# Image-Processing-Systems-Laboratory/DeepInPainting

Measured on AMD Instinct MI355X. Metric: train images/sec at 256x256, batch 8/GPU, 1/2/4/8 MI355X; IPSR layer ms, higher is better.
Workload: dtype f32; 1 GPU; BASELINE config 2: 256x256 synthetic images, 128x128 centre mask (M=256 of N=1024 feature positions), batch 8/GPU, fp32, full IPSR training step; global_batch=8, parallelism=dp1, dropout=True, conv_math=fp32, vgg16=seeded random init (no pretrained weights offline)

## Files before the change

### deepinpainting_amd/csrc/ipsr_common.h

```cpp
#pragma once
#include <hip/hip_runtime.h>
#include <stddef.h>
#include <stdint.h>

#include "../../include/ipsr_hip.h"

namespace ipsr {

void set_error(const char* fmt, ...);
int fail(int code, const char* fmt, ...);
int check_launch(const char* what);

void profile_mark_start(hipStream_t st, int region = 0);
void profile_mark_stop(hipStream_t st, int region = 0, double work = 0.0, double work2 = 0.0);

int debug_option(int key);

static inline size_t align_up(size_t v, size_t a) { return (v + a - 1) / a * a; }
static inline int cdiv(int a, int b) { return (a + b - 1) / b; }

struct Carver {
    char* base;
    size_t off;
    size_t cap;
    explicit Carver(void* p, size_t bytes) : base(static_cast<char*>(p)), off(0), cap(bytes) {}
    template <typename T>
    T* take(size_t count) {
        size_t start = align_up(off, 256);
        off = start + count * sizeof(T);
        return reinterpret_cast<T*>(base + start);
    }
    bool ok() const { return off <= cap; }
};

__device__ __forceinline__ unsigned xcd_remap(unsigned wg, unsigned nwg)
{
    const unsigned q = nwg >> 3, r = nwg & 7u;
    const unsigned xcd = wg & 7u, slot = wg >> 3;
    const unsigned start = xcd < r ? xcd * (q + 1u) : r * (q + 1u) + (xcd - r) * q;
    return start + slot;
}

__device__ __forceinline__ void remap2d(bool on, unsigned& bx, unsigned& by)
{
    bx = blockIdx.x; by = blockIdx.y;
    if (on) {
        const unsigned L = xcd_remap(blockIdx.x + gridDim.x * blockIdx.y, gridDim.x * gridDim.y);
        by = L / gridDim.x; bx = L - by * gridDim.x;
    }
}

struct CorrPartials {
    const float* pval;
    const int32_t* pidx;
    int ksplit;
};

__device__ __forceinline__ bool better(float v1, int i1, float v0, int i0)
{
    const bool n1 = v1 != v1, n0 = v0 != v0;
    return (v1 > v0) || (n1 && !n0) || ((v1 == v0 || (n1 && n0)) && i1 < i0);
}
__device__ __forceinline__ bool takes_over(float v, float best) { return (v > best) || (v != v && best == best); }

__device__ __forceinline__ void merged_argmax(const CorrPartials& cp, int b, int N, int q, float& v, int& i)
{
    const size_t base = (size_t)b * cp.ksplit * N + q;
    v = cp.pval[base];
    i = cp.pidx[base];
    for (int s = 1; s < cp.ksplit; ++s) {
        const float vs = cp.pval[base + (size_t)s * N];
        const int is = cp.pidx[base + (size_t)s * N];
        if (better(vs, is, v, i)) { v = vs; i = is; }
    }
    i = min(max(i, 0), N - 1);
}

typedef unsigned short bf16_t;
__device__ __forceinline__ float bf2f(bf16_t h) { return __uint_as_float((unsigned)h << 16); }
__device__ __forceinline__ bf16_t f2bf(float f)
{
    unsigned u = __float_as_uint(f);
    u += 0x7fffu + ((u >> 16) & 1u);
    return (bf16_t)(u >> 16);
}
__device__ __forceinline__ unsigned f2bf2(float lo, float hi) { return (unsigned)f2bf(lo) | ((unsigned)f2bf(hi) << 16); }
__device__ __forceinline__ float ld1(const float* p, size_t i) { return p[i]; }
__device__ __forceinline__ float ld1(const bf16_t* p, size_t i) { return bf2f(p[i]); }
__device__ __forceinline__ void st1(float* p, size_t i, float v) { p[i] = v; }
__device__ __forceinline__ void st1(bf16_t* p, size_t i, float v) { p[i] = f2bf(v); }
__device__ __forceinline__ float4 ld4(const float* p, size_t i4) { return reinterpret_cast<const float4*>(p)[i4]; }
__device__ __forceinline__ float4 ld4(const bf16_t* p, size_t i4)
{
    const uint2 r = reinterpret_cast<const uint2*>(p)[i4];
    return make_float4(__uint_as_float(r.x << 16), __uint_as_float(r.x & 0xffff0000u), __uint_as_float(r.y << 16),
                       __uint_as_float(r.y & 0xffff0000u));
}
__device__ __forceinline__ void st4(float* p, size_t i4, float4 v) { reinterpret_cast<float4*>(p)[i4] = v; }
__device__ __forceinline__ void st4(bf16_t* p, size_t i4, float4 v)
{
    uint2 r;
    r.x = (unsigned)f2bf(v.x) | ((unsigned)f2bf(v.y) << 16);
    r.y = (unsigned)f2bf(v.z) | ((unsigned)f2bf(v.w) << 16);
    reinterpret_cast<uint2*>(p)[i4] = r;
}

__device__ __forceinline__ int mpi_at(const int32_t* __restrict__ mpi, int l, int N)
{
    const int q = mpi[l];
    return q < 0 ? 0 : (q >= N ? N - 1 : q);
}

int launch_feat_mask(const uint8_t* mask, int H, int W, int layers, float threshold, uint8_t* feat,
                     void* ws, size_t ws_bytes, hipStream_t st);
int launch_index_prep(const uint8_t* feat, int h, int w, int patch, int stride, int mask_thred,
                      int32_t* flag, int32_t* mask_point_idx, int32_t* count, hipStream_t st);
int launch_patch_normalize(const float* x, int B, int C, int N, float* xn, float* xT, int Cp, float* inv,
                           hipStream_t st, int ldx = 0, int ldn = 0);
int launch_unfold(const float* x, int B, int C, int h, int w, int patch, int ld, float* xu, hipStream_t st);
int launch_fold(const float* yu, int B, int C, int h, int w, int patch, float* out, hipStream_t st, const float* addend = nullptr);
int launch_window_prepare(const float* x, int B, int C, int h, int w, int patch, float* n1, float* inv, float* xT, int Cp, hipStream_t st);
size_t window_corr_ws_bytes(int B, int Np);
int launch_window_corr_argmax(const float* R, const float* inv, int B, int h, int w, int patch, void* ws, size_t ws_bytes, hipStream_t st,
                              CorrPartials* partials);
size_t corr_argmax_ws_bytes(int B, int C, int N);
int launch_corr_argmax(const float* xn, const float* ref, int B, int C, int N, int32_t* ind, float* vmax,
                       float* S_out, void* ws, size_t ws_bytes, hipStream_t st, CorrPartials* partials = nullptr);

bool corr_bf16_supported(int C, int N);
size_t corr_argmax_bf16_ws_bytes(int B, int C, int N);
int launch_corr_argmax_bf16(const float* xn, const float* ref, int B, int C, int N, int32_t* ind, float* vmax,
                            void* ws, size_t ws_bytes, hipStream_t st, CorrPartials* partials = nullptr);
bool corr_R_bf16_supported(int C);
size_t corr_R_bf16_ws_bytes(int B, int C, int N);
int launch_corr_R_bf16(const float* x, const float* ref, int B, int C, int N, float* R, void* ws, size_t ws_bytes, hipStream_t st);

size_t conv_gemm_ws_bytes(int transposed, int B, int Cred, int M, int Hin, int Win, int Hout, int Wout, int k, int stride, int pad, int dil);
int launch_conv_gemm(bool transposed, bool w_cred_major, const float* x, const float* w, float* y, int B, int Cred, int M,
                     int Hin, int Win, int Hout, int Wout, int k, int stride, int pad, int dil, void* ws, size_t ws_bytes, hipStream_t st);

struct AttnArgs {
    const float* xT;
    const float* inv;
    int32_t* ind;
    float* vmax;
    CorrPartials part;
    const int32_t* mpi;
    int mpi_stride;
    const int32_t* mcount;
    int B, C, Cp, N, M, Mc;
    float* wn;
    float* wo;
    int32_t* kq;
    int32_t* jq;
    int32_t* dlist;
    int32_t* mprime;
    int32_t* rankflag;
    float* ac;
    float* attn;
    float* out;
    int32_t* bwd_index;
};
int launch_attention(const AttnArgs& a, hipStream_t st);
int attention_limits(int Cp, int N, int M, int Mc);

int launch_backward(const float* g, const int32_t* mpi, int M, const float* attn, const int32_t* bwd_index,
                    float triple_w, int B, int C, int N, float* gin, hipStream_t st, int identity = 1);

int launch_bias_act(void* x, const float* bias, int B, int C, int HW, int act, float slope, int io_bf16, void* y2, size_t y2_bstride,
                    unsigned* tickets, hipStream_t st);
int launch_bias_relu_pool2(const void* x, const float* bias, int B, int C, int H, int W, int io_bf16, void* y, hipStream_t st);
int launch_cat_relu_fwd(const void* y, const void* x, int B, int C1, int C2, int HW, int io_bf16, void* out, hipStream_t st);
int launch_cat_relu_bwd(const void* g, const void* out, int B, int C1, int C2, int HW, int io_bf16, void* dy, void* dx, hipStream_t st);

int launch_instnorm_act_fwd(const void* x, const float* bias, const float* gamma, const float* beta, float eps, int act, float slope,
                            int B, int C, int HW, int io_bf16, void* y, float* mean, float* rstd, size_t y_bstride, void* y2, size_t y2_bstride,
                            unsigned* tickets, hipStream_t st);
int launch_instnorm_act_bwd(const void* dy, const void* y, const void* x, const float* bias, const float* gamma, const float* mean,
                            const float* rstd, int act, float slope, int B, int C, int HW, int io_bf16, void* dx, float* dgamma_p,
                            float* dbeta_p, float* dbias_p, float* sums, unsigned* tickets, size_t dy_bstride, size_t y_bstride, const void* dy2,
                            size_t dy2_bstride, hipStream_t st);
int launch_bias_act_bwd(const void* dy, const void* y, int act, float slope, int B, int C, int HW, int io_bf16, void* dx, float* dbias_p,
                        float* sums, unsigned* tickets, const void* dy2, size_t dy2_bstride, hipStream_t st);

size_t innercos_ws_bytes(int B, int Cuse, int N);
int launch_innercos_loss(const float* x, int B, int Cx, int Cuse, int N, const float* mask, const float* target,
                         float strength, float* loss, void* ws, size_t ws_bytes, hipStream_t st);
int launch_innercos_loss_fused(const float* x, int B, int Cx, int Cuse, int N, const float* mask, const float* target, float strength, float* loss,
                               void* ws, size_t ws_bytes, unsigned* ticket, hipStream_t st);
int launch_innercos_backward(const float* x, int B, int Cx, int Cuse, int N, const float* mask,
                             const float* target, float strength, const float* grad_loss, float* grad_x,
                             hipStream_t st);

}
```

### deepinpainting_amd/csrc/winograd.hip

```cpp
#include <type_traits>

#include "ipsr_common.h"

namespace ipsr {

typedef float f32x16 __attribute__((ext_vector_type(16)));
typedef const __attribute__((address_space(1))) void* gptr_t;
typedef __attribute__((address_space(3))) void* lptr_t;

constexpr int WG_BM = 128, WG_BN = 128, WG_BK = 16, WG_NBUF = 4, WG_THREADS = 256;

struct WinoSplit {
    int nsplit, sps, xi_split, nsplit_t, sps_t;
    int nxi = 36;
    __host__ __device__ int slabs() const { return xi_split >= nxi ? nsplit : (xi_split <= 0 ? nsplit_t : (nsplit > nsplit_t ? nsplit : nsplit_t)); }
    __host__ __device__ int of(int xi) const { return xi < xi_split ? nsplit : nsplit_t; }
    __host__ __device__ int head_xi() const { return xi_split < nxi ? xi_split : nxi; }
    __host__ int workgroups(int tiles_per_xi) const { return tiles_per_xi * (head_xi() * nsplit + (nxi - head_xi()) * nsplit_t); }
};

__device__ __forceinline__ void wino_load_sum(const float* __restrict__ M, const WinoSplit sp, size_t plane, size_t off, float m[6][6])
{
#pragma unroll
    for (int i = 0; i < 6; ++i)
#pragma unroll
        for (int j = 0; j < 6; ++j) m[i][j] = M[(size_t)(i * 6 + j) * plane + off];
    const int nmin = sp.xi_split >= 36 ? sp.nsplit : (sp.nsplit < sp.nsplit_t ? sp.nsplit : sp.nsplit_t), nmax = sp.slabs();
    for (int s = 1; s < nmin; ++s) {
        const float* Ms = M + (size_t)s * 36 * plane;
#pragma unroll
        for (int i = 0; i < 6; ++i)
#pragma unroll
            for (int j = 0; j < 6; ++j) m[i][j] += Ms[(size_t)(i * 6 + j) * plane + off];
    }
    for (int s = nmin < 1 ? 1 : nmin; s < nmax; ++s) {
        const float* Ms = M + (size_t)s * 36 * plane;
#pragma unroll
        for (int i = 0; i < 6; ++i)
#pragma unroll
            for (int j = 0; j < 6; ++j)
                if (s < sp.of(i * 6 + j)) m[i][j] += Ms[(size_t)(i * 6 + j) * plane + off];
    }
}

__device__ __forceinline__ void wino_bt(const float d[6], float v[6])
{
    v[0] = 4.0f * d[0] - 5.0f * d[2] + d[4];
    v[1] = -4.0f * d[1] - 4.0f * d[2] + d[3] + d[4];
    v[2] = 4.0f * d[1] - 4.0f * d[2] - d[3] + d[4];
    v[3] = -2.0f * d[1] - d[2] + 2.0f * d[3] + d[4];
    v[4] = 2.0f * d[1] - d[2] - 2.0f * d[3] + d[4];
    v[5] = 4.0f * d[1] - 5.0f * d[3] + d[5];
}
__device__ __forceinline__ void wino_g(const float g[3], float u[6])
{
    u[0] = 0.25f * g[0];
    u[1] = (-1.0f / 6.0f) * (g[0] + g[1] + g[2]);
    u[2] = (-1.0f / 6.0f) * (g[0] - g[1] + g[2]);
    u[3] = (1.0f / 24.0f) * g[0] + (1.0f / 12.0f) * g[1] + (1.0f / 6.0f) * g[2];
    u[4] = (1.0f / 24.0f) * g[0] - (1.0f / 12.0f) * g[1] + (1.0f / 6.0f) * g[2];
    u[5] = g[2];
}
__device__ __forceinline__ void wino_at(const float m[6], float y[4])
{
    y[0] = m[0] + m[1] + m[2] + m[3] + m[4];
    y[1] = m[1] - m[2] + 2.0f * m[3] - 2.0f * m[4];
    y[2] = m[1] + m[2] + 4.0f * m[3] + 4.0f * m[4];
    y[3] = m[1] - m[2] + 8.0f * m[3] - 8.0f * m[4] + m[5];
}

__device__ __forceinline__ void wino_g4(const float e[4], float u[6])
{
    u[0] = 0.25f * e[0];
    u[1] = (-1.0f / 6.0f) * (e[0] + e[1] + e[2] + e[3]);
    u[2] = (-1.0f / 6.0f) * (e[0] - e[1] + e[2] - e[3]);
    u[3] = (1.0f / 24.0f) * e[0] + (1.0f / 12.0f) * e[1] + (1.0f / 6.0f) * e[2] + (1.0f / 3.0f) * e[3];
    u[4] = (1.0f / 24.0f) * e[0] - (1.0f / 12.0f) * e[1] + (1.0f / 6.0f) * e[2] - (1.0f / 3.0f) * e[3];
    u[5] = e[3];
}
__device__ __forceinline__ void wino_at3(const float m[6], float y[3])
{
    y[0] = m[0] + m[1] + m[2] + m[3] + m[4];
    y[1] = m[1] - m[2] + 2.0f * m[3] - 2.0f * m[4];
    y[2] = m[1] + m[2] + 4.0f * m[3] + 4.0f * m[4] + m[5];
}

typedef short bf16x8 __attribute__((ext_vector_type(8)));

constexpr int SPLIT_ROWS = 32;
constexpr int SPLIT_CHUNK = 12;
template <int NPL> constexpr int split_stage_elems() { return SPLIT_CHUNK * NPL * SPLIT_ROWS * 8; }

template <int NPL>
__device__ __forceinline__ void store_split(unsigned short* __restrict__ stage, const float (&v)[6][6], int pk, int rl,
                                            unsigned short* __restrict__ dst, size_t nblk, size_t rows, size_t blk, size_t row0)
{
    constexpr int NVEC = SPLIT_CHUNK * NPL * SPLIT_ROWS;
    const uint4* src = reinterpret_cast<const uint4*>(stage);
#pragma unroll
    for (int ch = 0; ch < 36 / SPLIT_CHUNK; ++ch) {
#pragma unroll
        for (int e = 0; e < SPLIT_CHUNK; ++e) {
            const int xi = ch * SPLIT_CHUNK + e;
            float r = v[xi / 6][xi % 6];
#pragma unroll
            for (int p = 0; p < NPL; ++p) {
                const unsigned short b = f2bf(r);
                stage[((e * NPL + p) * SPLIT_ROWS + rl) * 8 + pk] = b;
                r -= bf2f(b);
            }
        }
        __syncthreads();
#pragma unroll
        for (int it = 0; it < (NVEC + 255) / 256; ++it) {
            const int idx = threadIdx.x + it * 256;
            if (NVEC % 256 == 0 || idx < NVEC) {
                const int xp = idx / SPLIT_ROWS, r2 = idx - xp * SPLIT_ROWS;
                *reinterpret_cast<uint4*>(dst + (((size_t)(ch * SPLIT_CHUNK * NPL + xp) * nblk + blk) * rows + row0 + r2) * 8) = src[idx];
            }
        }
        __syncthreads();
    }
}

struct OpIdx { int t, c, pk, rl; unsigned bx, by; };

template <bool TMAJOR, int MODE> constexpr int op_smem_bytes()
{
    return MODE > 0 ? SPLIT_CHUNK * (MODE > 0 ? MODE : 1) * SPLIT_ROWS * 8 * 2 : (TMAJOR ? 36 * 16 * 17 * 4 : 16);
}

template <bool TMAJOR, int MODE>
__device__ __forceinline__ OpIdx op_index(unsigned bx, unsigned by)
{
    OpIdx ix;
    ix.bx = bx; ix.by = by;
    const int tid = threadIdx.x;
    if (!TMAJOR && MODE == 0) { ix.pk = 0; ix.rl = 0; ix.t = ix.bx * 256 + tid; ix.c = ix.by; }
    else if (!TMAJOR) { ix.pk = tid >> 5; ix.rl = tid & 31; ix.t = ix.bx * SPLIT_ROWS + ix.rl; ix.c = ix.by * 8 + ix.pk; }
    else if (MODE == 0) { ix.pk = tid & 15; ix.rl = tid >> 4; ix.t = ix.bx * 16 + ix.pk; ix.c = ix.by * 16 + ix.rl; }
    else { ix.pk = tid & 7; ix.rl = tid >> 3; ix.t = ix.bx * 8 + ix.pk; ix.c = ix.by * SPLIT_ROWS + ix.rl; }
    return ix;
}

static dim3 op_grid(bool tmajor, int mode, int Tp, int Cn)
{
    if (!tmajor) return mode == 0 ? dim3(cdiv(Tp, 256), Cn) : dim3(Tp / SPLIT_ROWS, Cn / 8);
    return mode == 0 ? dim3(Tp / 16, Cn / 16) : dim3(Tp / 8, Cn / SPLIT_ROWS);
}

__device__ __forceinline__ void wino_store_tmajor(float (*stage)[16][17], const float v[6][6], int tl, int cl, float* __restrict__ dst,
                                                  int t0, int c0, int Tp, int Cp);

template <bool TMAJOR, int MODE>
__device__ __forceinline__ void op_emit(unsigned char* smem, const float (&v)[6][6], const OpIdx& ix, void* __restrict__ out, int Cn, int Tp)
{
    if (MODE > 0) {
        unsigned short* stage = reinterpret_cast<unsigned short*>(smem);
        if (!TMAJOR) store_split<(MODE > 0 ? MODE : 1)>(stage, v, ix.pk, ix.rl, static_cast<unsigned short*>(out), Cn / 8, Tp, ix.by, (size_t)ix.bx * SPLIT_ROWS);
        else store_split<(MODE > 0 ? MODE : 1)>(stage, v, ix.pk, ix.rl, static_cast<unsigned short*>(out), Tp / 8, Cn, ix.bx, (size_t)ix.by * SPLIT_ROWS);
    } else if (TMAJOR) {
        wino_store_tmajor(reinterpret_cast<float (*)[16][17]>(smem), v, ix.pk, ix.rl, static_cast<float*>(out), ix.bx * 16, ix.by * 16, Tp, Cn);
    } else {
        float* V = static_cast<float*>(out);
        const size_t plane = (size_t)Cn * Tp;
#pragma unroll
        for (int i = 0; i < 6; ++i)
#pragma unroll
            for (int j = 0; j < 6; ++j) V[(size_t)(i * 6 + j) * plane + (size_t)ix.c * Tp + ix.t] = v[i][j];
    }
}

template <typename BODY>
__global__ void __launch_bounds__(256) wino_one_kernel(const BODY body, int remap)
{
    __shared__ __attribute__((aligned(16))) unsigned char smem[BODY::SMEM];
    unsigned bx, by;
    remap2d(remap != 0, bx, by);
    body(smem, bx, by);
}

template <typename BODY_A, typename BODY_B, int WAVES = 1>
__global__ void __launch_bounds__(256, WAVES) wino_pair_kernel(const BODY_A a, unsigned ax, const BODY_B b, unsigned bxn, unsigned n0, int swap, int remap)
{
    __shared__ __attribute__((aligned(16))) unsigned char smem[BODY_A::SMEM > BODY_B::SMEM ? BODY_A::SMEM : BODY_B::SMEM];
    unsigned id = blockIdx.x;
    const bool first = id < n0;
    if (first) { if (remap) id = xcd_remap(id, n0); }
    else id -= n0;
    if (first != (swap != 0)) {
        const unsigned y = id / ax;
        a(smem, id - y * ax, y);
        asm volatile("; end of part A" ::: "memory");
    } else {
        const unsigned y = id / bxn;
        b(smem, id - y * bxn, y);
        asm volatile("; end of part B" ::: "memory");
    }
}

static int wino_paired() { return !debug_option(2); }

template <typename BODY_A, typename BODY_B>
static void launch_two(hipStream_t st, const BODY_A& first, dim3 ga, int remap, const BODY_B& second, dim3 gb)
{
    wino_one_kernel<BODY_B><<<gb, 256, 0, st>>>(second, 0);
    wino_one_kernel<BODY_A><<<ga, 256, 0, st>>>(first, remap);
}

template <int WAVES = 1, typename BODY_A, typename BODY_B>
static void launch_pair(hipStream_t st, const BODY_A& first, dim3 ga, int remap, const BODY_B& second, dim3 gb, bool second_live = true)
{
    if (!second_live) { wino_one_kernel<BODY_A><<<ga, 256, 0, st>>>(first, remap); return; }
    if (!wino_paired()) return launch_two(st, first, ga, remap, second, gb);
    const unsigned na = ga.x * ga.y, nb = gb.x * gb.y;
    wino_pair_kernel<BODY_A, BODY_B, WAVES><<<na + nb, 256, 0, st>>>(first, ga.x, second, gb.x, na, 0, remap);
}

constexpr unsigned WRW_PAIR_MAX_SHORT = 4096;
template <typename BODY_A, typename BODY_B>
static void launch_pair_wrw(hipStream_t st, const BODY_A& a, dim3 ga, const BODY_B& b, dim3 gb, bool tile_may_lead)
// ... 561 lines not shown
    }
}

static int wino_rows_padded(int K, int math) { return (math == 0 && K <= 64) ? 64 : (K + WG_BM - 1) / WG_BM * WG_BM; }
static int wino_row_tiles(int Kp) { return Kp == 64 ? 1 : Kp / WG_BM; }

static int g_force_split[3] = {0, 0, 0};

static WinoSplit wino_choose_split(int tiles36, int stages, size_t m_bytes)
{
    const int tiles = tiles36 / 36;
    WinoSplit best{1, stages, 36, 1, stages};
    if (g_force_split[0] > 0) {
        const int a = g_force_split[0], x = g_force_split[1], b = g_force_split[2];
        if (a <= stages && b <= stages) {
            const int pa = cdiv(stages, a), pb = cdiv(stages, b);
            return WinoSplit{cdiv(stages, pa), pa, x, cdiv(stages, pb), pb};
        }
    }
    if (tiles36 <= 144 && stages <= 32) return best;
    if ((tiles == 8 || tiles == 16) && stages >= 16 && stages <= 128) {
        const int nt = stages >= 32 ? 4 : 2, per = cdiv(stages, nt);
        return WinoSplit{1, stages, 32, cdiv(stages, per), per};
    }
    double best_t = -1.0;
    const int cand[] = {1, 2, 3, 4, 6, 8, 12, 16};
    for (int ns : cand) {
        if (ns > 1 && stages / ns < 4) break;
        const int per = cdiv(stages, ns), real = cdiv(stages, per);
        const long wgs = (long)tiles36 * real;
        const long rounds = (wgs + 511) / 512;
        const long tail = wgs - (rounds - 1) * 512;
        double t = (rounds - 1) * (per + 3) * 1.7 + (per + 3) * (tail <= 256 ? 1.15 : 1.7);
        t += (real - 1) * (double)m_bytes * 2.0 / 4.0e6;
        if (best_t < 0.0 || t < best_t) { best_t = t; best = WinoSplit{real, per, 36, real, per}; }
    }
    return best;
}

struct ConvArith { int math; bool in_bf16, out_bf16; };
static inline bool arith_ok(const ConvArith& a) { return a.math == 0 || a.math == 2 || a.math == 3; }

template <typename F> static inline void with_mode(int math, F&& f)
{
    if (math == 2) f(std::integral_constant<int, 2>{});
    else if (math == 3) f(std::integral_constant<int, 3>{});
    else f(std::integral_constant<int, 0>{});
}
template <typename F> static inline void with_type(bool bf16, F&& f)
{
    if (bf16) f(static_cast<bf16_t*>(nullptr));
    else f(static_cast<float*>(nullptr));
}
#define ELEM_T(tag) std::remove_pointer_t<decltype(tag)>

struct WinoGemmPlan { int TY, TX, T, Tp, rows, cols, red; WinoSplit sp; size_t a_floats, b_floats, m_floats, total_bytes; };

static int round_up_bn(int n) { return (n + WG_BN - 1) / WG_BN * WG_BN; }

static void wino_plan_tiles(WinoGemmPlan* p, int B, int TY, int TX)
{
    p->TY = TY; p->TX = TX;
    p->T = B * TY * TX;
    p->Tp = round_up_bn(p->T);
}

static void wino_plan_gemm(WinoGemmPlan* p, int produced, int cols, int red, int math)
{
    p->rows = wino_rows_padded(produced, math);
    p->cols = cols;
    p->red = red;
    p->a_floats = (size_t)36 * red * p->rows * 3 / 2;
    p->b_floats = (size_t)36 * red * cols * 3 / 2;
    const size_t m1 = (size_t)36 * p->rows * cols;
    p->sp = wino_choose_split(36 * wino_row_tiles(p->rows) * (cols / WG_BN), red / WG_BK, m1 * 4);
    p->m_floats = m1 * p->sp.slabs();
    p->total_bytes = align_up(p->a_floats * 4, 256) + align_up(p->b_floats * 4, 256) + align_up(p->m_floats * 4, 256) + 256;
}

template <typename F> static size_t wino_ws_bytes(F&& plan)
{
    WinoGemmPlan p, q;
    if (plan(&p, -1) != IPSR_OK || plan(&q, 0) != IPSR_OK) return 0;
    return p.total_bytes > q.total_bytes ? p.total_bytes : q.total_bytes;
}

struct WinoBufs { float *A, *B, *M; };
static int no_check() { return IPSR_OK; }

template <typename Check = int (*)()>
static int wino_launch_head(const char* who, const char* arith_note, const WinoGemmPlan& p, const ConvArith& ar, void* ws, size_t ws_bytes,
                            WinoBufs* b, Check family_check = no_check)
{
    if (ws_bytes < p.total_bytes) return fail(IPSR_ERR_WORKSPACE, "%s: workspace %zu < %zu", who, ws_bytes, p.total_bytes);
    if (int rc = family_check()) return rc;
    if (!arith_ok(ar)) return fail(IPSR_ERR_INVALID, "%s: arithmetic %d%s", who, ar.math, arith_note);
    Carver cv(ws, ws_bytes);
    b->A = cv.take<float>(p.a_floats);
    b->B = cv.take<float>(p.b_floats);
    b->M = cv.take<float>(p.m_floats);
    return IPSR_OK;
}

static int wino_remap() { return !debug_option(1); }

static int launch_wino_gemm(int math, const WinoGemmPlan& p, const WinoBufs& b, hipStream_t st, double useful)
{
    const int kt = wino_row_tiles(p.rows), tt = p.cols / WG_BN;
    const unsigned grid = p.sp.workgroups(kt * tt);
    const unsigned short *As = reinterpret_cast<const unsigned short*>(b.A), *Bs = reinterpret_cast<const unsigned short*>(b.B);
    profile_mark_start(st, 3);
    if (math == 2)
        wino_gemm_split_kernel<2><<<grid, WG_THREADS, 0, st>>>(As, Bs, p.red, p.rows, p.cols, kt, tt, p.sp, b.M);
    else if (math == 3)
        wino_gemm_split_kernel<3><<<grid, WG_THREADS, 0, st>>>(As, Bs, p.red, p.rows, p.cols, kt, tt, p.sp, b.M);
    else if (p.rows == 64)
        wino_gemm_kernel<64><<<grid, WG_THREADS, 0, st>>>(b.A, b.B, p.red, p.rows, p.cols, kt, tt, p.sp, b.M);
    else
        wino_gemm_kernel<128><<<grid, WG_THREADS, 0, st>>>(b.A, b.B, p.red, p.rows, p.cols, kt, tt, p.sp, b.M);
    profile_mark_stop(st, 3, 72.0 * p.red * p.rows * p.cols, useful);
    return check_launch("wino_gemm_kernel");
}

static int wino_plan(int B, int C, int K, int H, int W, WinoGemmPlan* p, int math)
{
    if (C % WG_BK != 0) return fail(IPSR_ERR_UNSUPPORTED, "winograd: %d reduction channels are not a multiple of %d", C, WG_BK);
    wino_plan_tiles(p, B, (H + 3) / 4, (W + 3) / 4);
    wino_plan_gemm(p, K, p->Tp, C, math);
    return IPSR_OK;
}

size_t winograd_ws_bytes(int B, int C, int K, int H, int W)
{
    return wino_ws_bytes([&](WinoGemmPlan* p, int math) { return wino_plan(B, C, K, H, W, p, math); });
}

size_t winograd_filter_floats(int C, int K) { return (size_t)36 * C * ((K + WG_BM - 1) / WG_BM * WG_BM) * 3 / 2; }

int launch_winograd(const void* x, const float* w, void* y, int B, int C, int K, int H, int W, long sc, long sm, int flip,
                    void* ws, size_t ws_bytes, hipStream_t st, const float* bias = nullptr, int epilogue = 0,
                    float* u_cache = nullptr, int u_valid = 0, ConvArith ar = ConvArith{0, false, false})
{
    WinoGemmPlan p;
    WinoBufs m;
    if (int rc = wino_plan(B, C, K, H, W, &p, ar.math)) return rc;
    auto epilogue_ok = [&] {
        if (epilogue < 0 || epilogue > 2 || (epilogue == 2 && ((H | W) & 1)))
            return fail(IPSR_ERR_INVALID, "winograd: epilogue %d on a %dx%d map", epilogue, H, W);
        return (int)IPSR_OK;
    };
    if (int rc = wino_launch_head("winograd", " (0 = fp32 MFMA, 2 / 3 = split bf16)", p, ar, ws, ws_bytes, &m, epilogue_ok)) return rc;
    if (u_cache) m.A = u_cache;
    const int remap = wino_remap();
    with_mode(ar.math, [&](auto M) {
        constexpr int MODE = decltype(M)::value;
        with_type(ar.in_bf16, [&](auto* tag) {
            using T = ELEM_T(tag);
            launch_pair(st, WinoInput<MODE, T>{static_cast<const T*>(x), B, C, H, W, p.TY, p.TX, p.Tp, m.B}, op_grid(false, MODE, p.Tp, C), remap,
                        WinoFilter<MODE>{w, C, K, p.rows, sc, sm, flip, m.A}, op_grid(false, MODE, p.rows, C), !(u_cache && u_valid));
        });
    });
    if (int rc = check_launch("wino_pair_kernel<WinoInput, WinoFilter>")) return rc;
    if (int rc = launch_wino_gemm(ar.math, p, m, st, 72.0 * C * K * p.T)) return rc;
    const dim3 og(cdiv(p.T, 256), K);
    with_type(ar.out_bf16, [&](auto* tag) {
        using T = ELEM_T(tag);
        T* yo = static_cast<T*>(y);
        if (epilogue == 2) wino_output_kernel<2, T><<<og, 256, 0, st>>>(m.M, p.sp, bias, B, K, p.rows, H, W, p.TY, p.TX, p.Tp, yo, remap);
        else if (epilogue == 1) wino_output_kernel<1, T><<<og, 256, 0, st>>>(m.M, p.sp, bias, B, K, p.rows, H, W, p.TY, p.TX, p.Tp, yo, remap);
        else wino_output_kernel<0, T><<<og, 256, 0, st>>>(m.M, p.sp, bias, B, K, p.rows, H, W, p.TY, p.TX, p.Tp, yo, remap);
    });
    return check_launch("wino_output_kernel");
}

static int wino_wrw_plan(int B, int K, int C, int H, int W, WinoGemmPlan* p, int math)
{
    wino_plan_tiles(p, B, (H + 3) / 4, (W + 3) / 4);
    wino_plan_gemm(p, K, round_up_bn(C), p->Tp, math);
    return IPSR_OK;
}

size_t winograd_wrw_ws_bytes(int B, int K, int C, int H, int W)
{
    return wino_ws_bytes([&](WinoGemmPlan* p, int math) { return wino_wrw_plan(B, K, C, H, W, p, math); });
}

int launch_winograd_wrw(const void* et, const void* dt, float* dW, int B, int K, int C, int H, int W, void* ws, size_t ws_bytes, hipStream_t st,
                        ConvArith ar = ConvArith{0, false, false})
{
    WinoGemmPlan p;
    WinoBufs m;
    wino_wrw_plan(B, K, C, H, W, &p, ar.math);
    if (int rc = wino_launch_head("winograd wrw", "", p, ar, ws, ws_bytes, &m)) return rc;
    with_mode(ar.math, [&](auto M) {
        constexpr int MODE = decltype(M)::value;
        with_type(ar.in_bf16, [&](auto* tag) {
            using T = ELEM_T(tag);
            launch_pair_wrw(st, WinoWrwTile<MODE, T>{static_cast<const T*>(et), B, K, H, W, p.TY, p.TX, p.Tp, p.rows, m.A}, op_grid(true, MODE, p.Tp, p.rows),
                            WinoWrwWindow<MODE, T>{static_cast<const T*>(dt), B, C, H, W, p.TY, p.TX, p.Tp, p.cols, m.B}, op_grid(true, MODE, p.Tp, p.cols),
                            MODE != 3);
        });
    });
    if (int rc = check_launch("wino_pair_kernel<WinoWrwTile, WinoWrwWindow>")) return rc;
    if (int rc = launch_wino_gemm(ar.math, p, m, st, 72.0 * p.T * K * C)) return rc;
    wino_wrw_output_kernel<<<dim3(cdiv(C, 256), K), 256, 0, st>>>(m.M, p.sp, K, C, p.rows, p.cols, dW);
    return check_launch("wino_wrw_output_kernel");
}


template <int OS, int IS, bool TMAJOR, int MODE, typename TIN>
struct WinoWindow {
    const TIN* x; int B, C, H, Wd, off, TY, TX, Tp, Cp; void* V;
    static constexpr int SMEM = op_smem_bytes<TMAJOR, MODE>();
    __device__ __forceinline__ void operator()(unsigned char* smem, unsigned bx, unsigned by) const
    {
    const OpIdx ix = op_index<TMAJOR, MODE>(bx, by);
    const int t = ix.t, c = ix.c;
    if (!TMAJOR && MODE == 0 && t >= Tp) return;
    const int T = B * TY * TX;
    const bool live = t < T && c < C;
    int b = 0, ty = 0, tx = 0;
    if (live) { b = t / (TY * TX); const int rem = t - b * TY * TX; ty = rem / TX; tx = rem - ty * TX; }
    const TIN* xp = x + ((size_t)b * C + (live ? c : 0)) * H * Wd;
    float d[6][6];
#pragma unroll
    for (int i = 0; i < 6; ++i) {
        const int yy = IS * (OS * ty + i) + off;
        const bool yok = live && (unsigned)yy < (unsigned)H;
#pragma unroll
        for (int j = 0; j < 6; ++j) {
            const int xx = IS * (OS * tx + j) + off;
            d[i][j] = (yok && (unsigned)xx < (unsigned)Wd) ? ld1(xp, (size_t)yy * Wd + xx) : 0.0f;
        }
    }
    float w[6][6], v[6][6];
#pragma unroll
    for (int j = 0; j < 6; ++j) {
        const float col[6] = {d[0][j], d[1][j], d[2][j], d[3][j], d[4][j], d[5][j]};
        float o[6];
        wino_bt(col, o);
#pragma unroll
        for (int i = 0; i < 6; ++i) w[i][j] = o[i];
    }
#pragma unroll
    for (int i = 0; i < 6; ++i) wino_bt(w[i], v[i]);
    op_emit<TMAJOR, MODE>(smem, v, ix, V, TMAJOR ? Cp : C, Tp);
    }
};

template <int MODE>
struct Wino4Filter {
    const float* W; int C, K, Kp; long sc, sm; int flip; void* U;
    static constexpr int SMEM = MODE > 0 ? op_smem_bytes<false, MODE>() : 256 * 17 * 4;
    __device__ __forceinline__ void operator()(unsigned char* smem, unsigned bx, unsigned by) const
    {
    const OpIdx ix = op_index<false, MODE>(bx, by);
    const int k = ix.t, c = ix.c;
    float g[4][4];
    if (MODE == 0 && sm == 16) {
        float* taps = reinterpret_cast<float*>(smem);
        const int k0 = bx * 256, n = (K - k0 < 256 ? K - k0 : 256) * 16;
        const float* src = W + (long)c * sc + (long)k0 * 16;
        for (int i = threadIdx.x; i < n; i += 256) taps[(i >> 4) * 17 + (i & 15)] = src[i];
        __syncthreads();
        if (k >= Kp) return;
#pragma unroll
        for (int r = 0; r < 4; ++r)
#pragma unroll
            for (int s2 = 0; s2 < 4; ++s2) {
                const int rr = flip ? 3 - r : r, ss = flip ? 3 - s2 : s2;
                g[r][s2] = k < K ? taps[threadIdx.x * 17 + rr * 4 + ss] : 0.0f;
            }
    } else {
        if (MODE == 0 && k >= Kp) return;
#pragma unroll
        for (int r = 0; r < 4; ++r)
#pragma unroll
            for (int s2 = 0; s2 < 4; ++s2) {
                const int rr = flip ? 3 - r : r, ss = flip ? 3 - s2 : s2;
                g[r][s2] = k < K ? W[(long)c * sc + (long)k * sm + rr * 4 + ss] : 0.0f;
            }
    }
    float t[6][4], u[6][6];
#pragma unroll
    for (int s2 = 0; s2 < 4; ++s2) {
        const float col[4] = {g[0][s2], g[1][s2], g[2][s2], g[3][s2]};
        float o[6];
        wino_g4(col, o);
#pragma unroll
        for (int i = 0; i < 6; ++i) t[i][s2] = o[i];
    }
#pragma unroll
    for (int i = 0; i < 6; ++i) wino_g4(t[i], u[i]);
    op_emit<false, MODE>(smem, u, ix, U, C, Kp);
    }
};

template <typename TOUT>
__global__ void __launch_bounds__(256) wino3_output_kernel(const float* __restrict__ Mo, WinoSplit split, int B, int K, int Kp, int Ho, int Wo,
                                                           int TY, int TX, int Tp, int Hy, int Wy, int os, int oo, TOUT* __restrict__ y)
{
    const int t = blockIdx.x * 256 + threadIdx.x, k = blockIdx.y;
    const int T = B * TY * TX;
    if (t >= T) return;
    float m[6][6];
    const size_t plane = (size_t)Kp * Tp;
// ... 720 lines not shown
```

Measured before the change: 359.5 images/sec.

## Add fused Winograd kernel for narrow-output fp32 convolutions

Adds a single kernel that loads input windows, applies the Winograd input transform into LDS, runs fp32 MFMA against pre-transformed filters, and applies the output transform with optional bias/ReLU/maxpool in registers. It is used for fp32 convs with K<=64 and C divisible by 16 when the tile count is large. This removes the global round trips of the transformed-input and product tensors and the separate input, GEMM and output launches. In exchange it keeps 72 accumulator vectors per thread at one workgroup per CU, which risks register pressure and low occupancy.

Result: faster. 365.5 images/sec (median of 6 runs) (+1.6%).

```diff
diff --git a/deepinpainting_amd/csrc/ipsr_common.h b/deepinpainting_amd/csrc/ipsr_common.h
--- a/deepinpainting_amd/csrc/ipsr_common.h
+++ b/deepinpainting_amd/csrc/ipsr_common.h
@@ -135,6 +135,9 @@
 size_t corr_R_bf16_ws_bytes(int B, int C, int N);
 int launch_corr_R_bf16(const float* x, const float* ref, int B, int C, int N, float* R, void* ws, size_t ws_bytes, hipStream_t st);
 
+bool wino_fused_admits(int math, bool in_bf16, bool out_bf16, int B, int C, int K, int H, int W);
+int launch_wino_fused(const float* x, const float* U, const float* bias, float* y, int B, int C, int K, int H, int W, int epilogue, hipStream_t st);
+
 size_t conv_gemm_ws_bytes(int transposed, int B, int Cred, int M, int Hin, int Win, int Hout, int Wout, int k, int stride, int pad, int dil);
 int launch_conv_gemm(bool transposed, bool w_cred_major, const float* x, const float* w, float* y, int B, int Cred, int M,
                      int Hin, int Win, int Hout, int Wout, int k, int stride, int pad, int dil, void* ws, size_t ws_bytes, hipStream_t st);
diff --git a/deepinpainting_amd/csrc/wino_fused.hip b/deepinpainting_amd/csrc/wino_fused.hip
--- /dev/null
+++ b/deepinpainting_amd/csrc/wino_fused.hip
@@ -0,0 +1,232 @@
+#include "ipsr_common.h"
+#include "wino_transforms.h"
+
+namespace ipsr {
+
+typedef float f32x4 __attribute__((ext_vector_type(4)));
+
+constexpr int WF_THREADS = 256;
+constexpr int WF_TROWS = 2, WF_TCOLS = 16, WF_TILES = WF_TROWS * WF_TCOLS;
+constexpr int WF_CK = 16;
+constexpr int WF_KP = 64;
+constexpr int WF_PF = 4;
+constexpr int WF_LDS_BYTES = 36 * WF_CK * WF_TILES * 4;
+constexpr long WF_MIN_TILES = 8192;
+
+template <bool VEC>
+__device__ __forceinline__ void wf_load_window(const float* __restrict__ xp, bool live, int y0, int x0, int H, int Wd, float (&d)[6][6])
+{
+#pragma unroll
+    for (int i = 0; i < 6; ++i) {
+        const int yy = y0 + i;
+        const bool yok = live && (unsigned)yy < (unsigned)H;
+        if (VEC) {
+            const float* rp = xp + (size_t)(yok ? yy : 0) * Wd;
+            const float4 mid = yok ? ld4(rp, (size_t)(x0 + 1) >> 2) : make_float4(0.f, 0.f, 0.f, 0.f);
+            d[i][0] = (yok && x0 >= 0) ? rp[x0] : 0.0f;
+            d[i][1] = mid.x; d[i][2] = mid.y; d[i][3] = mid.z; d[i][4] = mid.w;
+            d[i][5] = (yok && x0 + 5 < Wd) ? rp[x0 + 5] : 0.0f;
+        } else {
+#pragma unroll
+            for (int j = 0; j < 6; ++j) {
+                const int xx = x0 + j;
+                d[i][j] = (yok && (unsigned)xx < (unsigned)Wd) ? xp[(size_t)yy * Wd + xx] : 0.0f;
+            }
+        }
+    }
+}
+
+__device__ __forceinline__ void wf_transform_store(const float (&d)[6][6], float* __restrict__ Vc)
+{
+    float w[6][6], v[6];
+#pragma unroll
+    for (int j = 0; j < 6; ++j) {
+        const float col[6] = {d[0][j], d[1][j], d[2][j], d[3][j], d[4][j], d[5][j]};
+        float o[6];
+        wino_bt(col, o);
+#pragma unroll
+        for (int i = 0; i < 6; ++i) w[i][j] = o[i];
+    }
+#pragma unroll
+    for (int i = 0; i < 6; ++i) {
+        wino_bt(w[i], v);
+#pragma unroll
+        for (int j = 0; j < 6; ++j) Vc[(i * 6 + j) * WF_CK * WF_TILES] = v[j];
+    }
+}
+
+template <int EPI, bool VEC>
+__global__ void __launch_bounds__(WF_THREADS, 1) wino_fused_kernel(const float* __restrict__ x, const float* __restrict__ U, const float* __restrict__ bias,
+                                                                    float* __restrict__ y, int C, int K, int H, int Wd, int TY, int TX, int nbx, int nby)
+{
+    extern __shared__ __attribute__((aligned(16))) float V[];
+    const int tid = threadIdx.x, lane = tid & 63, wave = __builtin_amdgcn_readfirstlane(tid >> 6);
+    unsigned id = blockIdx.x;
+    const int bx = id % nbx;
+    id /= nbx;
+    const int by = id % nby, b = id / nby;
+    const size_t HW = (size_t)H * Wd;
+
+    const int tl = tid & 31, tc = tid >> 5;
+    const int wty = WF_TROWS * by + (tl >> 4), wtx = WF_TCOLS * bx + (tl & 15);
+    const bool live = wty < TY && wtx < TX;
+    const int wy0 = 4 * wty - 1, wx0 = 4 * wtx - 1;
+    const float* xw = x + ((size_t)b * C + tc) * HW;
+    float* Vw = V + tc * WF_TILES + (tl ^ ((tc & 1) << 4));
+
+    const int kq = lane >> 4, ln = lane & 15;
+    const float* Ua = U + (size_t)kq * WF_KP + 16 * wave + ln;
+    const float* Vb0 = V + kq * WF_TILES + (ln ^ ((kq & 1) << 4));
+    const float* Vb1 = V + kq * WF_TILES + ((16 + ln) ^ ((kq & 1) << 4));
+    const size_t uplane = (size_t)C * WF_KP;
+
+    f32x4 acc[36][2];
+#pragma unroll
+    for (int xi = 0; xi < 36; ++xi)
+#pragma unroll
+        for (int h = 0; h < 2; ++h) acc[xi][h] = f32x4{0.0f, 0.0f, 0.0f, 0.0f};
+
+    float raw[2][6][6];
+    if (VEC) {
+        wf_load_window<VEC>(xw, live, wy0, wx0, H, Wd, raw[0]);
+        wf_load_window<VEC>(xw + 8 * HW, live, wy0, wx0, H, Wd, raw[1]);
+    }
+
+    const int nchunk = C / WF_CK;
+    for (int ch = 0; ch < nchunk; ++ch) {
+        const float* Uc = Ua + (size_t)ch * WF_CK * WF_KP;
+        float ua[36][4];
+#pragma unroll
+        for (int xi = 0; xi < WF_PF; ++xi)
+#pragma unroll
+            for (int g = 0; g < 4; ++g) ua[xi][g] = Uc[xi * uplane + g * 4 * WF_KP];
+
+        const float* xc = xw + (size_t)ch * WF_CK * HW;
+        if (!VEC) wf_load_window<VEC>(xc, live, wy0, wx0, H, Wd, raw[0]);
+        wf_transform_store(raw[0], Vw);
+        if (!VEC) wf_load_window<VEC>(xc + 8 * HW, live, wy0, wx0, H, Wd, raw[1]);
+        wf_transform_store(raw[1], Vw + 8 * WF_TILES);
+        __syncthreads();
+
+        if (VEC && ch + 1 < nchunk) {
+            wf_load_window<VEC>(xc + WF_CK * HW, live, wy0, wx0, H, Wd, raw[0]);
+            wf_load_window<VEC>(xc + (WF_CK + 8) * HW, live, wy0, wx0, H, Wd, raw[1]);
+        }
+
+#pragma unroll
+        for (int xi = 0; xi < 36; ++xi) {
+            if (xi + WF_PF < 36) {
+#pragma unroll
+                for (int g = 0; g < 4; ++g) ua[xi + WF_PF][g] = Uc[(xi + WF_PF) * uplane + g * 4 * WF_KP];
+            }
+            float vb[4][2];
+#pragma unroll
+            for (int g = 0; g < 4; ++g) {
+                vb[g][0] = Vb0[(xi * WF_CK + 4 * g) * WF_TILES];
+                vb[g][1] = Vb1[(xi * WF_CK + 4 * g) * WF_TILES];
+            }
+#pragma unroll
+            for (int g = 0; g < 4; ++g) {
+                acc[xi][0] = __builtin_amdgcn_mfma_f32_16x16x4f32(ua[xi][g], vb[g][0], acc[xi][0], 0, 0, 0);
+                acc[xi][1] = __builtin_amdgcn_mfma_f32_16x16x4f32(ua[xi][g], vb[g][1], acc[xi][1], 0, 0, 0);
+            }
+        }
+        __syncthreads();
+    }
+
+    const int tx = WF_TCOLS * bx + ln;
+#pragma unroll
+    for (int h = 0; h < 2; ++h) {
+        const int ty = WF_TROWS * by + h;
+#pragma unroll
+        for (int r = 0; r < 4; ++r) {
+            const int k = 16 * wave + 4 * kq + r;
+            float w[4][6], o[4][4];
+#pragma unroll
+            for (int j = 0; j < 6; ++j) {
+                const float col[6] = {acc[j][h][r], acc[6 + j][h][r], acc[12 + j][h][r], acc[18 + j][h][r], acc[24 + j][h][r], acc[30 + j][h][r]};
+                float r4[4];
+                wino_at(col, r4);
+#pragma unroll
+                for (int i = 0; i < 4; ++i) w[i][j] = r4[i];
+            }
+#pragma unroll
+            for (int i = 0; i < 4; ++i) wino_at(w[i], o[i]);
+            if (k >= K || ty >= TY || tx >= TX) continue;
+            if (EPI >= 1) {
+                const float bv = bias ? bias[k] : 0.0f;
+#pragma unroll
+                for (int i = 0; i < 4; ++i)
+#pragma unroll
+                    for (int j = 0; j < 4; ++j) { const float v = o[i][j] + bv; o[i][j] = v < 0.0f ? 0.0f : v; }
+            }
+            if (EPI == 2) {
+                const int Hh = H >> 1, Wh = Wd >> 1;
+                float* yp = y + ((size_t)b * K + k) * Hh * Wh;
+#pragma unroll
+                for (int i = 0; i < 2; ++i) {
+                    float pm[2];
+#pragma unroll
+                    for (int j = 0; j < 2; ++j) {
+                        const float a0 = o[2 * i][2 * j], a1 = o[2 * i][2 * j + 1], a2 = o[2 * i + 1][2 * j], a3 = o[2 * i + 1][2 * j + 1];
+                        const float m01 = (a0 > a1 || a0 != a0) ? a0 : a1, m23 = (a2 > a3 || a2 != a2) ? a2 : a3;
+                        pm[j] = (m01 > m23 || m01 != m01) ? m01 : m23;
+                    }
+                    const int yy = 2 * ty + i, xx = 2 * tx;
+                    if (yy >= Hh) continue;
+                    if (VEC) {
+                        *reinterpret_cast<float2*>(yp + (size_t)yy * Wh + xx) = make_float2(pm[0], pm[1]);
+                    } else {
+                        if (xx < Wh) yp[(size_t)yy * Wh + xx] = pm[0];
+                        if (xx + 1 < Wh) yp[(size_t)yy * Wh + xx + 1] = pm[1];
+                    }
+                }
+                continue;
+            }
+            float* yp = y + ((size_t)b * K + k) * HW;
+            const int y0 = 4 * ty, x0 = 4 * tx;
+#pragma unroll
+            for (int i = 0; i < 4; ++i) {
+                if (y0 + i >= H) continue;
+                if (VEC) {
+                    st4(yp, ((size_t)(y0 + i) * Wd + x0) >> 2, make_float4(o[i][0], o[i][1], o[i][2], o[i][3]));
+                } else {
+#pragma unroll
+                    for (int j = 0; j < 4; ++j)
+                        if (x0 + j < Wd) yp[(size_t)(y0 + i) * Wd + x0 + j] = o[i][j];
+                }
+            }
+        }
+    }
+}
+
+bool wino_fused_admits(int math, bool in_bf16, bool out_bf16, int B, int C, int K, int H, int W)
+{
+    const int opt = debug_option(7);
+    if (opt == 1 || math != 0 || in_bf16 || out_bf16 || K > WF_KP || C % WF_CK != 0) return false;
+    if (opt == 2) return true;
+    return (long)B * ((H + 3) / 4) * ((W + 3) / 4) >= WF_MIN_TILES;
+}
+
+template <int EPI, bool VEC>
+static int wf_launch(const float* x, const float* U, const float* bias, float* y, int B, int C, int K, int H, int W, hipStream_t st)
+{
+    const int TY = (H + 3) / 4, TX = (W + 3) / 4;
+    const int nbx = cdiv(TX, WF_TCOLS), nby = cdiv(TY, WF_TROWS);
+    const hipError_t e = hipFuncSetAttribute(reinterpret_cast<const void*>(&wino_fused_kernel<EPI, VEC>), hipFuncAttributeMaxDynamicSharedMemorySize, WF_LDS_BYTES);
+    if (e != hipSuccess) return fail(IPSR_ERR_LAUNCH, "wino_fused_kernel: hipFuncSetAttribute(dynamic LDS %d): %s", WF_LDS_BYTES, hipGetErrorString(e));
+    wino_fused_kernel<EPI, VEC><<<(unsigned)((size_t)B * nby * nbx), WF_THREADS, WF_LDS_BYTES, st>>>(x, U, bias, y, C, K, H, W, TY, TX, nbx, nby);
+    return check_launch("wino_fused_kernel");
+}
+
+int launch_wino_fused(const float* x, const float* U, const float* bias, float* y, int B, int C, int K, int H, int W, int epilogue, hipStream_t st)
+{
+    if ((size_t)B * cdiv((H + 3) / 4, WF_TROWS) * cdiv((W + 3) / 4, WF_TCOLS) > 0x7fffffffu)
+        return fail(IPSR_ERR_UNSUPPORTED, "wino_fused_kernel: too many tile blocks");
+    const bool vec = (W & 3) == 0;
+    if (epilogue == 2) return vec ? wf_launch<2, true>(x, U, bias, y, B, C, K, H, W, st) : wf_launch<2, false>(x, U, bias, y, B, C, K, H, W, st);
+    if (epilogue == 1) return vec ? wf_launch<1, true>(x, U, bias, y, B, C, K, H, W, st) : wf_launch<1, false>(x, U, bias, y, B, C, K, H, W, st);
+    return vec ? wf_launch<0, true>(x, U, bias, y, B, C, K, H, W, st) : wf_launch<0, false>(x, U, bias, y, B, C, K, H, W, st);
+}
+
+}
diff --git a/deepinpainting_amd/csrc/wino_transforms.h b/deepinpainting_amd/csrc/wino_transforms.h
--- /dev/null
+++ b/deepinpainting_amd/csrc/wino_transforms.h
@@ -0,0 +1,22 @@
+#pragma once
+
+namespace ipsr {
+
+__device__ __forceinline__ void wino_bt(const float d[6], float v[6])
+{
+    v[0] = 4.0f * d[0] - 5.0f * d[2] + d[4];
+    v[1] = -4.0f * d[1] - 4.0f * d[2] + d[3] + d[4];
+    v[2] = 4.0f * d[1] - 4.0f * d[2] - d[3] + d[4];
+    v[3] = -2.0f * d[1] - d[2] + 2.0f * d[3] + d[4];
+    v[4] = 2.0f * d[1] - d[2] - 2.0f * d[3] + d[4];
+    v[5] = 4.0f * d[1] - 5.0f * d[3] + d[5];
+}
+__device__ __forceinline__ void wino_at(const float m[6], float y[4])
+{
+    y[0] = m[0] + m[1] + m[2] + m[3] + m[4];
+    y[1] = m[1] - m[2] + 2.0f * m[3] - 2.0f * m[4];
+    y[2] = m[1] + m[2] + 4.0f * m[3] + 4.0f * m[4];
+    y[3] = m[1] - m[2] + 8.0f * m[3] - 8.0f * m[4] + m[5];
+}
+
+}
diff --git a/deepinpainting_amd/csrc/winograd.hip b/deepinpainting_amd/csrc/winograd.hip
--- a/deepinpainting_amd/csrc/winograd.hip
+++ b/deepinpainting_amd/csrc/winograd.hip
@@ -1,6 +1,7 @@
 #include <type_traits>
 
 #include "ipsr_common.h"
+#include "wino_transforms.h"
 
 namespace ipsr {
 
@@ -43,15 +44,6 @@
     }
 }
 
-__device__ __forceinline__ void wino_bt(const float d[6], float v[6])
-{
-    v[0] = 4.0f * d[0] - 5.0f * d[2] + d[4];
-    v[1] = -4.0f * d[1] - 4.0f * d[2] + d[3] + d[4];
-    v[2] = 4.0f * d[1] - 4.0f * d[2] - d[3] + d[4];
-    v[3] = -2.0f * d[1] - d[2] + 2.0f * d[3] + d[4];
-    v[4] = 2.0f * d[1] - d[2] - 2.0f * d[3] + d[4];
-    v[5] = 4.0f * d[1] - 5.0f * d[3] + d[5];
-}
 __device__ __forceinline__ void wino_g(const float g[3], float u[6])
 {
     u[0] = 0.25f * g[0];
@@ -60,13 +52,6 @@
     u[3] = (1.0f / 24.0f) * g[0] + (1.0f / 12.0f) * g[1] + (1.0f / 6.0f) * g[2];
     u[4] = (1.0f / 24.0f) * g[0] - (1.0f / 12.0f) * g[1] + (1.0f / 6.0f) * g[2];
     u[5] = g[2];
-}
-__device__ __forceinline__ void wino_at(const float m[6], float y[4])
-{
-    y[0] = m[0] + m[1] + m[2] + m[3] + m[4];
-    y[1] = m[1] - m[2] + 2.0f * m[3] - 2.0f * m[4];
-    y[2] = m[1] + m[2] + 4.0f * m[3] + 4.0f * m[4];
-    y[3] = m[1] - m[2] + 8.0f * m[3] - 8.0f * m[4] + m[5];
 }
 
 __device__ __forceinline__ void wino_g4(const float e[4], float u[6])
@@ -934,6 +919,13 @@
     if (int rc = wino_launch_head("winograd", " (0 = fp32 MFMA, 2 / 3 = split bf16)", p, ar, ws, ws_bytes, &m, epilogue_ok)) return rc;
     if (u_cache) m.A = u_cache;
     const int remap = wino_remap();
+    if (wino_fused_admits(ar.math, ar.in_bf16, ar.out_bf16, B, C, K, H, W)) {
+        if (!(u_cache && u_valid)) {
+            wino_one_kernel<WinoFilter<0>><<<op_grid(false, 0, p.rows, C), 256, 0, st>>>(WinoFilter<0>{w, C, K, p.rows, sc, sm, flip, m.A}, 0);
+            if (int rc = check_launch("wino_one_kernel<WinoFilter>")) return rc;
+        }
+        return launch_wino_fused(static_cast<const float*>(x), m.A, bias, static_cast<float*>(y), B, C, K, H, W, epilogue, st);
+    }
     with_mode(ar.math, [&](auto M) {
         constexpr int MODE = decltype(M)::value;
         with_type(ar.in_bf16, [&](auto* tag) {
```
